# cinemere/evacuation

Measured on AMD Instinct MI355X. Metric: env-steps/s (agent-updates/s) at n=60x4096 envs, higher is better.
Workload: dtype f32

## Files before the change

evacuation_amd/csrc/evac_families.h:

```cpp
#pragma once

#include <type_traits>

#include "evac_common.h"

namespace evac {


template <int WPE_, int BLOCK1_ = 256>
struct Wave {
    static constexpr int WPE = WPE_;
    static constexpr bool kEnvUniform = true;
    static constexpr int kThreadsPerEnv = WPE * kWave;
    static constexpr int kBlock = (WPE == 1 || BLOCK1_ == 1024) ? (BLOCK1_ > kThreadsPerEnv ? BLOCK1_ : kThreadsPerEnv) : kThreadsPerEnv;
    static constexpr int kEnvsPerBlock = kBlock / kThreadsPerEnv;
    static constexpr bool kPace = kBlock == 1024 && kEnvsPerBlock > 1;
    static constexpr bool kEnvBarrier = WPE > 1 && kEnvsPerBlock > 1;
    static constexpr bool kHelpers = false, kExitLane = true, kPipelined = false;
    static constexpr const char* kName = WPE == 1 ? (kPace ? "1 wave/env, all pairs, CU-wide workgroups" : "1 wave/env, all pairs") : (WPE == 2 ? "2 waves/env, all pairs" : (WPE == 4 ? (kPace ? "4 waves/env, all pairs, CU-wide workgroups" : "4 waves/env, all pairs") : (WPE == 8 ? "8 waves/env, all pairs" : "16 waves/env, all pairs")));

    static constexpr int kTiles = WPE == 1 ? 1 : 2;
    static constexpr int kRows = WPE == 1 ? 1 : (WPE == 2 ? 2 : 4);
    static constexpr int kPairs = WPE * kWave / 2;

    struct Smem {
        f4 tile[kTiles][kEnvsPerBlock][WPE * kWave];
        float2 rowpos[kTiles][kEnvsPerBlock][WPE == 1 ? 1 : WPE * kWave];
        float2 part[kRows][kEnvsPerBlock][WPE == 1 ? 1 : WPE * kWave];
        f4 redf[kEnvsPerBlock][WPE];
        i4 redi[kEnvsPerBlock][WPE];
        int cols[kEnvsPerBlock][WPE];
        float exitg[kEnvsPerBlock][2];
        int poison[2][kEnvsPerBlock];
        int bar[kEnvsPerBlock];
        int persist_cmd[kEnvsPerBlock][6];
        alignas(16) float stage[kEnvsPerBlock][kStageSteps][12];
        alignas(16) int progress[kPace ? 16 : 4];
        int pace_sink[kPace ? 16 : 1][kPace ? kWave : 1];
        int deal_hist[kPace ? kWave + 2 : 1];
        int chain_ok[kEnvsPerBlock];
    };

    struct Ctx {
        using Family = Wave<WPE_, BLOCK1_>;
        Smem& sm;
        int env, slot, wave_in_env, lane, i;
        bool owner;
        int par = 0, next_cols = 0, next_base = 0, next_rows = 0, next_rbase = 0;
        bool have_next = false;
        __device__ __forceinline__ explicit Ctx(Smem& s) : sm(s) {
            const int t = threadIdx.x;
            slot = t / kThreadsPerEnv;
            const int tin = t - slot * kThreadsPerEnv;
            wave_in_env = tin / kWave;
            lane = tin & (kWave - 1);
            i = tin;
            env = blockIdx.x * kEnvsPerBlock + slot;
            if constexpr (WPE == 1) {
                env = __builtin_amdgcn_readfirstlane(env);
                slot = __builtin_amdgcn_readfirstlane(slot);
            }
            owner = i == 0;
        }
    };

    static __device__ __forceinline__ void sync() {
        static_assert(!kEnvBarrier, "several multi-wave envs per workgroup: use sync(ctx)");
        if constexpr (WPE == 1) {
            __builtin_amdgcn_fence(__ATOMIC_ACQ_REL, "wavefront");
            __builtin_amdgcn_wave_barrier();
        } else {
            __syncthreads();
        }
    }
    template <class C>
    static __device__ __forceinline__ void sync(C& c) {
        if constexpr (!kEnvBarrier) {
            sync();
        } else {
            __builtin_amdgcn_fence(__ATOMIC_RELEASE, "workgroup");
            if (c.lane == 0) {
                int* ctr = &c.sm.bar[c.slot];
                const int old = __hip_atomic_fetch_add(ctr, 1, __ATOMIC_RELAXED, __HIP_MEMORY_SCOPE_WORKGROUP);
                const int target = (old & ~(WPE - 1)) + WPE;
                int spins = 0;
                while (__hip_atomic_load(ctr, __ATOMIC_RELAXED, __HIP_MEMORY_SCOPE_WORKGROUP) < target && ++spins < (1 << 24)) __builtin_amdgcn_s_sleep(0);
            }
            __builtin_amdgcn_fence(__ATOMIC_ACQUIRE, "workgroup");
            __builtin_amdgcn_wave_barrier();
        }
    }

    static __device__ __forceinline__ void init(Ctx& c) {
        if constexpr (WPE > 1) {
            if (c.wave_in_env == 0 && c.lane < 2) c.sm.poison[c.lane][c.slot] = 0;
            if (c.wave_in_env == 0 && c.lane == 2) c.sm.bar[c.slot] = 0;
            __syncthreads();
        }
    }
    static __device__ __forceinline__ void invalidate(Ctx& c) { c.have_next = false; }
    static __device__ __forceinline__ bool aborted(Ctx&) { return false; }

    template <bool GUARD, class C>
    static __device__ __forceinline__ void reduce(const Params&, C& c, Sums& s, const unsigned long long (&pred)[8]) {
        wave_sum3(s.f0, s.f1, s.f2);
#pragma unroll
        for (int k = 0; k < 8; ++k) s.i[k] = mask_count(pred[k]);
        if constexpr (WPE > 1) {
            auto& sm = c.sm;
            if constexpr (GUARD) C::Family::sync(c);
            if (c.lane == 0) {
                sm.redf[c.slot][c.wave_in_env] = f4{s.f0, s.f1, s.f2, 0.0f};
                sm.redi[c.slot][c.wave_in_env] = i4{s.i[0] | (s.i[1] << 16), s.i[2] | (s.i[3] << 16), s.i[4] | (s.i[5] << 16), s.i[6] | (s.i[7] << 16)};
            }
            C::Family::sync(c);
            const int w = c.lane < WPE ? c.lane : WPE - 1;
            f4 rf = sm.redf[c.slot][w];
            i4 ri = sm.redi[c.slot][w];
#define EVAC_RED_STEP(CTRL)                                                                                      \
    rf.x = dpp_add<CTRL, 0xf>(rf.x); rf.y = dpp_add<CTRL, 0xf>(rf.y); rf.z = dpp_add<CTRL, 0xf>(rf.z);           \
    ri.x = dpp_addi<CTRL, 0xf>(ri.x); ri.y = dpp_addi<CTRL, 0xf>(ri.y); ri.z = dpp_addi<CTRL, 0xf>(ri.z);        \
    ri.w = dpp_addi<CTRL, 0xf>(ri.w);
            EVAC_RED_STEP(0x111)
            if constexpr (WPE > 2) { EVAC_RED_STEP(0x112) }
            if constexpr (WPE > 4) { EVAC_RED_STEP(0x114) }
            if constexpr (WPE > 8) { EVAC_RED_STEP(0x118) }
#undef EVAC_RED_STEP
            s.f0 = readlane_f(rf.x, WPE - 1);
            s.f1 = readlane_f(rf.y, WPE - 1);
            s.f2 = readlane_f(rf.z, WPE - 1);
            if constexpr (!GUARD && std::is_same<typename C::Family, Wave>::value) {
                const int wi = __builtin_amdgcn_readfirstlane(c.wave_in_env);
                const int before = wi == 0 ? 0 : __builtin_amdgcn_readlane(ri.y, max(wi - 1, 0));
                c.next_base = before >> 16;
                c.next_cols = __builtin_amdgcn_readlane(ri.y, WPE - 1) >> 16;
                const int rbefore = wi == 0 ? 0 : __builtin_amdgcn_readlane(ri.z, max(wi - 1, 0));
                c.next_rbase = rbefore >> 16;
                c.next_rows = __builtin_amdgcn_readlane(ri.z, WPE - 1) >> 16;
                c.have_next = true;
            }
            const int a = __builtin_amdgcn_readlane(ri.x, WPE - 1), b = __builtin_amdgcn_readlane(ri.y, WPE - 1);
            const int d = __builtin_amdgcn_readlane(ri.z, WPE - 1), g = __builtin_amdgcn_readlane(ri.w, WPE - 1);
            s.i[0] = a & 0xffff; s.i[1] = a >> 16;
            s.i[2] = b & 0xffff; s.i[3] = b >> 16;
            s.i[4] = d & 0xffff; s.i[5] = d >> 16;
            s.i[6] = g & 0xffff; s.i[7] = g >> 16;
        }
    }

    template <class C>
    static __device__ __forceinline__ void exit_publish(C& c, bool exit_lane, float gx, float gy) {
        if constexpr (WPE > 1) {
            if (exit_lane) {
                c.sm.exitg[c.slot][0] = gx;
                c.sm.exitg[c.slot][1] = gy;
            }
        }
    }
    template <class C>
    static __device__ __forceinline__ void exit_fetch(C& c, float gx, float gy, int src_i, float& ex, float& ey) {
        if constexpr (WPE == 1) {
            ex = readlane_f(gx, src_i);
            ey = readlane_f(gy, src_i);
        } else {
            ex = c.sm.exitg[c.slot][0];
            ey = c.sm.exitg[c.slot][1];
        }
    }

    static __device__ __forceinline__ void neighbour_sum(const Params& p, Ctx& c, const Ped& q, bool efv, bool fv,
                                                         float ux, float uy, float& sx, float& sy) {
        auto& sm = c.sm;
        int par = 0;
        if constexpr (WPE == 1) {
            sx = 0.0f;
            sy = 0.0f;
            if (ballot(fv) == 0ull) {
                if ((ballot(ux != ux || uy != uy) & ballot(efv)) != 0ull) sx = sy = __builtin_nanf("");
                return;
            }
            sync(c);
        } else {
            par = c.par;
            c.par = par ^ 1;
        }
        int n_cols, n_rows = 0, row_rank = 0;
        unsigned long long moving_mask;
        {
            const unsigned long long m = moving_mask = ballot(efv);
            int before = __builtin_amdgcn_mbcnt_hi((unsigned)(m >> 32), __builtin_amdgcn_mbcnt_lo((unsigned)m, 0u));
            n_cols = __popcll(m);
            if constexpr (WPE > 1) {
                const unsigned long long mr = ballot(fv);
                row_rank = __builtin_amdgcn_mbcnt_hi((unsigned)(mr >> 32), __builtin_amdgcn_mbcnt_lo((unsigned)mr, 0u));
                n_rows = __popcll(mr);
                if (c.have_next) {
                    n_cols = c.next_cols;
                    before += c.next_base;
                    n_rows = c.next_rows;
                    row_rank += c.next_rbase;
                } else {
                    if (c.lane == 0) sm.cols[c.slot][c.wave_in_env] = n_cols | (n_rows << 16);
                    sync(c);
                    int tot = 0, base = 0;
#pragma unroll
                    for (int w2 = 0; w2 < WPE; ++w2) {
                        const int k = sm.cols[c.slot][w2];
                        base += (w2 < c.wave_in_env) ? k : 0;
                        tot += k;
                    }
                    n_cols = tot & 0xffff;
                    before += base & 0xffff;
                    n_rows = tot >> 16;
                    row_rank += base >> 16;
                }
            }
            const int tid = c.wave_in_env * kWave + c.lane;
            const int idx = efv ? before : n_cols + (tid - before);
            if constexpr (WPE == 1) {
                float* tf = (float*)sm.tile[par][c.slot] + (idx >> 1) * 4 + (idx & 1);
                tf[0] = efv ? q.x * kTileScale : __builtin_inff();
                tf[2] = q.y * kTileScale;
                tf[kPairs * 4 + 0] = efv ? ux : 0.0f;
                tf[kPairs * 4 + 2] = efv ? uy : 0.0f;
            } else {
                sm.tile[par][c.slot][idx] = f4{efv ? q.x * kTileScale : __builtin_inff(), q.y * kTileScale, efv ? ux : 0.0f, efv ? uy : 0.0f};
            }
        }
        if constexpr (WPE > 1) {
            if (fv) sm.rowpos[par][c.slot][row_rank] = make_float2(q.x * kTileScale, q.y * kTileScale);
            if ((ballot(ux != ux || uy != uy) & moving_mask) != 0ull && c.lane == 0) sm.poison[par][c.slot] = 1;
        }
        sync(c);
        bool poisoned = false;
        if constexpr (WPE > 1) {
            poisoned = sm.poison[par][c.slot] != 0;
            if (c.wave_in_env == 0 && c.lane == 0) sm.poison[par ^ 1][c.slot] = 0;
        }
        sx = 0.0f;
        sy = 0.0f;
        const f4* __restrict__ tile = sm.tile[par][c.slot];
        const float r2b = kRPed2Big;
        if constexpr (WPE == 1) {
            const int n8 = __builtin_amdgcn_readfirstlane((n_cols + 3) & ~3);
            const float XI = q.x * kTileScale, YI = q.y * kTileScale;
            constexpr int B = 16;
            const f2 P = f2{XI, YI}, r2b2 = f2{r2b, r2b};
            f2 sx2 = f2{0.0f, 0.0f}, sy2 = f2{0.0f, 0.0f};
            const f4* __restrict__ txy = tile;
            const f4* __restrict__ tuv = tile + kPairs;
            int m = 0;
            const int mp = n8 >> 1;
            for (; m + B / 2 <= mp; m += B / 2) {
                f4 a[B / 2], u[B / 2];
#pragma unroll
                for (int k = 0; k < B / 2; ++k) { a[k] = txy[m + k]; u[k] = tuv[m + k]; }
#pragma unroll
                for (int k = 0; k < B / 2; ++k) pair2_accumulate(P, a[k], u[k], r2b2, sx2, sy2);
            }
            if (mp - m >= 4) {
                f4 a[4], u[4];
#pragma unroll
                for (int k = 0; k < 4; ++k) { a[k] = txy[m + k]; u[k] = tuv[m + k]; }
#pragma unroll
                for (int k = 0; k < 4; ++k) pair2_accumulate(P, a[k], u[k], r2b2, sx2, sy2);
                m += 4;
            }
            if (m < mp) {
                f4 a[2], u[2];
#pragma unroll
                for (int k = 0; k < 2; ++k) { a[k] = txy[m + k]; u[k] = tuv[m + k]; }
#pragma unroll
                for (int k = 0; k < 2; ++k) pair2_accumulate(P, a[k], u[k], r2b2, sx2, sy2);
            }
            sx = hsum2(sx2);
            sy = hsum2(sy2);
        } else {
            const unsigned wu = (unsigned)__builtin_amdgcn_readfirstlane(c.wave_in_env);
            const unsigned nc = (unsigned)__builtin_amdgcn_readfirstlane(n_cols), nr = (unsigned)__builtin_amdgcn_readfirstlane(n_rows);
            const unsigned share_u = wu % (unsigned)kRows, first_row = (wu - share_u) * (unsigned)kWave;
            const int share = (int)share_u, gbase = (int)first_row + c.lane;
            const int slices = nr > first_row ? (int)min((nr - first_row + (unsigned)kWave - 1u) / (unsigned)kWave, (unsigned)kRows) : 0;
            const unsigned groups = (nc + 3u) >> 2;
            const unsigned per = (groups + (unsigned)kRows - 1u) / (unsigned)kRows;
            const int jbeg = (int)(share_u * per * 4u);
            const int jend = (int)(min((share_u + 1u) * per, groups) * 4u);
            auto sweep = [&](auto r_tag) {
                constexpr int R = decltype(r_tag)::value;
                constexpr int R2 = R / 2;
                float X[R], Y[R], ax[R], ay[R];
                f2 X2[R2 ? R2 : 1], Y2[R2 ? R2 : 1], ax2[R2 ? R2 : 1], ay2[R2 ? R2 : 1];
#pragma unroll
                for (int r = 0; r < R; ++r) {
                    const float2 rp = sm.rowpos[par][c.slot][gbase + r * kWave];
                    X[r] = rp.x; Y[r] = rp.y;
                    ax[r] = 0.0f; ay[r] = 0.0f;
                }
#pragma unroll
                for (int r = 0; r < R2; ++r) {
                    X2[r] = f2{X[2 * r], X[2 * r + 1]}; Y2[r] = f2{Y[2 * r], Y[2 * r + 1]};
                    ax2[r] = f2{0.0f, 0.0f}; ay2[r] = f2{0.0f, 0.0f};
                }
                const f2 r2b2 = f2{r2b, r2b};
                auto column = [&](f4 t) {
#pragma unroll
                    for (int r = 0; r < R2; ++r) pair_accumulate_rows2(X2[r], Y2[r], t, r2b2, ax2[r], ay2[r]);
#pragma unroll
                    for (int r = 2 * R2; r < R; ++r) pair_accumulate(X[r], Y[r], t, r2b, ax[r], ay[r]);
                };
                constexpr int B = (R <= 2 && !(kEnvBarrier && R == 2)) ? 8 : 4;
                int j = jbeg;
                for (; j + B <= jend; j += B) {
                    f4 t[B];
#pragma unroll
                    for (int k = 0; k < B; ++k) t[k] = tile[j + k];
#pragma unroll
                    for (int k = 0; k < B; ++k) column(t[k]);
                }
                if constexpr (B == 8) {
                    if (j < jend) {
                        f4 t[4];
#pragma unroll
                        for (int k = 0; k < 4; ++k) t[k] = tile[j + k];
#pragma unroll
                        for (int k = 0; k < 4; ++k) column(t[k]);
                    }
                }
#pragma unroll
                for (int r = 0; r < R2; ++r) { ax[2 * r] = ax2[r].x; ax[2 * r + 1] = ax2[r].y; ay[2 * r] = ay2[r].x; ay[2 * r + 1] = ay2[r].y; }
#pragma unroll
                for (int r = 0; r < R; ++r) sm.part[share][c.slot][gbase + r * kWave] = make_float2(ax[r], ay[r]);
            };
            if (slices == 1) sweep(std::integral_constant<int, 1>{});
            else if (slices == 2) sweep(std::integral_constant<int, 2>{});
            else if constexpr (kRows == 4) {
                if (slices == 3) sweep(std::integral_constant<int, 3>{});
                else if (slices == 4) sweep(std::integral_constant<int, 4>{});
            }
            sync(c);
            if (fv) {
#pragma unroll
                for (int r = 0; r < kRows; ++r) {
                    const float2 pr = sm.part[r][c.slot][row_rank];
                    sx += pr.x;
                    sy += pr.y;
                }
            }
            if (poisoned) sx = sy = __builtin_nanf("");
        }
    }
};

template <int WPE_>
struct Cells {
    static constexpr int WPE = WPE_;
    static_assert(WPE >= 2, "Cells is a workgroup-per-env family");
    static constexpr bool kEnvUniform = true;
    static constexpr int kThreadsPerEnv = WPE * kWave;
    static constexpr int kBlock = kThreadsPerEnv;
    static constexpr int kEnvsPerBlock = 1;
    static constexpr bool kPace = false, kHelpers = false, kExitLane = true, kPipelined = false, kEnvBarrier = false;
    static constexpr int kPad = 8;
    static constexpr int kRowBatch = 8;
    static constexpr int kTransposedWork = 1024;
    static constexpr const char* kName = WPE == 2 ? "2 waves/env, cell list" : (WPE == 4 ? "4 waves/env, cell list" : (WPE == 8 ? "8 waves/env, cell list" : "16 waves/env, cell list"));

    struct Smem {
        f4 tile[1][kThreadsPerEnv + kPad];
        alignas(16) int cnt[kCells + 4];
        alignas(16) int start[kCells + 4];
        int who[kThreadsPerEnv];
        int rowlist[kThreadsPerEnv];
        i2 res[kThreadsPerEnv];
        char one_workgroup_per_cu[WPE == 16 ? 52 * 1024 : 16];
        f4 redf[1][WPE];
        i4 redi[1][WPE];
        float exitg[1][2];
        alignas(16) float stage[1][kStageSteps][12];
    };

    struct Ctx {
        using Family = Cells<WPE_>;
        Smem& sm;
        int env, slot, wave_in_env, lane, i;
        bool owner;
        __device__ __forceinline__ explicit Ctx(Smem& s) : sm(s) {
            const int t = threadIdx.x;
            slot = 0;
            wave_in_env = t / kWave;
            lane = t & (kWave - 1);
            i = t;
            env = blockIdx.x;
            owner = i == 0;
        }
    };

    static __device__ __forceinline__ void sync() { __syncthreads(); }
    template <class C>
    static __device__ __forceinline__ void sync(C&) { __syncthreads(); }

    static __device__ __forceinline__ void invalidate(Ctx&) {}
    static __device__ __forceinline__ bool aborted(Ctx&) { return false; }
    static __device__ __forceinline__ void init(Ctx& c) {
        for (int k = c.i; k < kCells + 4; k += kThreadsPerEnv) c.sm.cnt[k] = 0;
        __syncthreads();
    }

    template <bool GUARD, class C>
    static __device__ __forceinline__ void reduce(const Params& p, C& c, Sums& s, const unsigned long long (&pred)[8]) {
        Wave<WPE>::template reduce<GUARD>(p, c, s, pred);
    }
    template <class C>
    static __device__ __forceinline__ void exit_publish(C& c, bool exit_lane, float gx, float gy) {
        Wave<WPE>::exit_publish(c, exit_lane, gx, gy);
    }
    template <class C>
    static __device__ __forceinline__ void exit_fetch(C& c, float gx, float gy, int src_i, float& ex, float& ey) {
        Wave<WPE>::exit_fetch(c, gx, gy, src_i, ex, ey);
    }

    static __device__ __forceinline__ int cell_of(const Params& p, float x, float y) {
        int cx = (int)((x + p.cell_ox) * p.cell_inv_hx), cy = (int)((y + p.cell_oy) * p.cell_inv_hy);
        cx = min(max(cx, 0), kCellsX - 1);
        cy = min(max(cy, 0), kCellsY - 1);
        return cx * kCellsY + cy;
    }

    static __device__ __forceinline__ void neighbour_sum(const Params& p, Ctx& c, const Ped& q, bool efv, bool fv,
                                                         float ux, float uy, float& sx, float& sy) {
        auto& sm = c.sm;
        const int cell = cell_of(p, q.x, q.y);
        int ticket = 0;
        if (efv) {
            ticket = atomicAdd(&sm.cnt[cell], 1);
            if (ux != ux || uy != uy) atomicAdd(&sm.cnt[kCells], 1);
        }
        __syncthreads();
        if (c.wave_in_env == 0) {
            const i4 v = *(const i4*)&sm.cnt[4 * c.lane];
            const int p1 = v.x, p2 = p1 + v.y, p3 = p2 + v.z, tot = p3 + v.w;
            const int incl = wave_inclusive_scan(tot);
            const int ex = incl - tot;
            *(i4*)&sm.start[4 * c.lane] = i4{ex, ex + p1, ex + p2, ex + p3};
            *(i4*)&sm.cnt[4 * c.lane] = i4{0, 0, 0, 0};
            if (c.lane == kWave - 1) {
                sm.start[kCells] = incl;
                sm.start[kCells + 1] = sm.cnt[kCells];
                sm.cnt[kCells] = 0;
                sm.cnt[kCells + 1] = 0;
            }
        }
        __syncthreads();
        const int n_cols = sm.start[kCells];
        const int n_nan = sm.start[kCells + 1];
        if (efv) {
            const int s = sm.start[cell] + ticket;
            const float hs = p.head_scale;
            const int hx = (int)__builtin_rintf(ux * hs), hy = (int)__builtin_rintf(uy * hs);
            sm.tile[0][s] = f4{q.x * kTileScale, q.y * kTileScale, __builtin_bit_cast(float, hx), __builtin_bit_cast(float, hy)};
            sm.who[s] = c.i | (fv ? 0x8000 : 0) | (cell << 16);
            if (fv) sm.rowlist[atomicAdd(&sm.cnt[kCells + 1], 1)] = s;
        }
        if (c.i < kPad) sm.tile[0][n_cols + c.i] = f4{__builtin_inff(), 0.0f, 0.0f, 0.0f};
        __syncthreads();
        const int n_need = __builtin_amdgcn_readfirstlane(sm.cnt[kCells + 1]);
        const int n_cols_u = __builtin_amdgcn_readfirstlane(n_cols);
        const bool transposed = n_need * ((n_cols_u + kWave - 1) / kWave) <= kTransposedWork;
          if (transposed) {
            const f4* __restrict__ tile = sm.tile[0];
            const int wv = __builtin_amdgcn_readfirstlane(c.wave_in_env);
            for (int k = wv; k < n_need; k += WPE) {
                const int s = sm.rowlist[k];
                const f4 me = tile[s];
                const int ped = sm.who[s] & 0x7fff;
                int ax = 0, ay = 0;
                for (int j0 = 0; j0 < n_cols_u; j0 += kWave)
                    pair_accumulate_int(me.x, me.y, tile[min(j0 + c.lane, n_cols_u)], kRPed2Big, ax, ay);
                wave_sum2_int_lane63(ax, ay);
                if (c.lane == kWave - 1) sm.res[ped] = i2{ax, ay};
            }
          } else {
            const int s = c.i;
            const int wc = s < n_cols ? sm.who[s] : 0;
            if (wc & 0x8000) {
                const f4 me = sm.tile[0][s];
                const int rc = wc >> 16;
                int lo[3], hi[3];
#pragma unroll
                for (int r = 0; r < 3; ++r) {
                    const int c0 = rc + (r - 1) * kCellsY - 1;
                    lo[r] = sm.start[min(max(c0, 0), kCells)];
                    hi[r] = sm.start[min(max(c0 + 3, 0), kCells)];
                }
                int ax = 0, ay = 0;
                int j = lo[0];
                const f4* __restrict__ tile = sm.tile[0];
#pragma unroll
                for (int r = 0; r < 3; ++r) {
                    j = max(j, lo[r]);
                    while (j < hi[r]) {
                        f4 t[kRowBatch];
#pragma unroll
                        for (int k = 0; k < kRowBatch; ++k) t[k] = tile[j + k];
#pragma unroll
                        for (int k = 0; k < kRowBatch; ++k) pair_accumulate_int(me.x, me.y, t[k], kRPed2Big, ax, ay);
                        j += kRowBatch;
                    }
                }
                sm.res[wc & 0x7fff] = i2{ax, ay};
            }
          }
        __syncthreads();
        const i2 r = sm.res[c.i];
        sx = fv ? (float)r.x : 0.0f;
        sy = fv ? (float)r.y : 0.0f;
        if (n_nan != 0) sx = sy = __builtin_nanf("");
    }
};

template <int G_, int BLOCK_ = 256>
struct Sub {
    static constexpr int G = G_;
    static_assert(G == 16 || G == 32, "sub-wave groups are 16 or 32 lanes");
    static constexpr bool kEnvUniform = false, kHelpers = false, kExitLane = true, kPipelined = false, kEnvBarrier = false;
    static constexpr int kThreadsPerEnv = G;
    static constexpr int kEnvsPerWave = kWave / G;
    static constexpr int kBlock = BLOCK_;
    static constexpr int kEnvsPerBlock = (kBlock / kWave) * kEnvsPerWave;
    static constexpr unsigned long long kGroupBits = G == 32 ? 0xffffffffull : 0xffffull;
    static constexpr const char* kName = G == 16 ? "4 envs/wave, all pairs" : "2 envs/wave, all pairs";

    struct Smem {
        f4 tile[kEnvsPerBlock][G];
    };

    struct Ctx {
        Smem& sm;
        int env, slot, lane, sub, i, li;
        unsigned long long gmask;
        bool owner;
        __device__ __forceinline__ explicit Ctx(Smem& s) : sm(s) {
            const int t = threadIdx.x;
            lane = t & (kWave - 1);
            sub = lane / G;
            li = i = lane - sub * G;
            slot = (t / kWave) * kEnvsPerWave + sub;
            env = blockIdx.x * kEnvsPerBlock + slot;
            gmask = kGroupBits << (sub * G);
            owner = li == G - 1;
        }
    };

    static __device__ __forceinline__ void sync() {
        __builtin_amdgcn_fence(__ATOMIC_ACQ_REL, "wavefront");
        __builtin_amdgcn_wave_barrier();
    }
    static __device__ __forceinline__ int count(unsigned long long m, unsigned long long gmask) { return __popcll(m & gmask); }
    static __device__ __forceinline__ int rank(unsigned long long m, unsigned long long gmask) {
        const unsigned long long g = m & gmask;
        return __builtin_amdgcn_mbcnt_hi((unsigned)(g >> 32), __builtin_amdgcn_mbcnt_lo((unsigned)g, 0u));
    }
    static __device__ __forceinline__ float fetch(float v, int sub_base, int src_i) { return __shfl(v, sub_base + src_i, kWave); }

    static __device__ __forceinline__ void invalidate(Ctx&) {}
    static __device__ __forceinline__ bool aborted(Ctx&) { return false; }
    template <bool GUARD, class C>
    static __device__ __forceinline__ void reduce(const Params&, C& c, Sums& s, const unsigned long long (&pred)[8]) {
        float &a = s.f0, &b = s.f1, &cc = s.f2;
        {
            float& c = cc;
            EVAC_DPP3(0x111, 0xf)
            EVAC_DPP3(0x112, 0xf)
            EVAC_DPP3(0x114, 0xf)
            EVAC_DPP3(0x118, 0xf)
            if constexpr (G == 32) { EVAC_DPP3(0x142, 0xa) }
        }
#pragma unroll
        for (int k = 0; k < 8; ++k) s.i[k] = count(pred[k], c.gmask);
    }
    template <class C>
    static __device__ __forceinline__ void exit_publish(C&, bool, float, float) {}
    template <class C>
    static __device__ __forceinline__ void exit_fetch(C& c, float gx, float gy, int src_i, float& ex, float& ey) {
        ex = fetch(gx, c.sub * G, src_i);
        ey = fetch(gy, c.sub * G, src_i);
    }

    static __device__ __forceinline__ void neighbour_sum(const Params& p, Ctx& c, const Ped& q, bool efv, bool fv,
                                                         float ux, float uy, float& sx, float& sy) {
        auto& sm = c.sm;
        sync();
        const unsigned long long m_efv = ballot(efv);
        const int n_cols = count(m_efv, c.gmask);
        {
            const int before = rank(m_efv, c.gmask);
            const int idx = efv ? before : n_cols + (c.li - before);
            float* tf = (float*)sm.tile[c.slot] + (idx >> 1) * 8 + (idx & 1);
            tf[0] = efv ? q.x * kTileScale : __builtin_inff();
            tf[2] = q.y * kTileScale;
            tf[4] = efv ? ux : 0.0f;
            tf[6] = efv ? uy : 0.0f;
        }
        sync();
        sx = 0.0f;
        sy = 0.0f;
        int nmax = 0;
#pragma unroll
        for (int g = 0; g < kEnvsPerWave; ++g) {
            const int k = __popcll((m_efv >> (g * G)) & kGroupBits);
            nmax = k > nmax ? k : nmax;
        }
        const bool any_row = ballot(fv) != 0ull;
        const int n4 = any_row ? ((nmax + 3) & ~3) : 0;
        if (!any_row) {
            const unsigned long long m_nan = ballot(ux != ux || uy != uy) & m_efv;
            if ((m_nan & c.gmask) != 0ull) sx = sy = __builtin_nanf("");
        }
        const f4* __restrict__ tile = sm.tile[c.slot];
        const float XI = q.x * kTileScale, YI = q.y * kTileScale;
        int j = 0;
        const f2 P = f2{XI, YI}, r2b2 = f2{kRPed2Big, kRPed2Big};
        f2 sx2 = f2{0.0f, 0.0f}, sy2 = f2{0.0f, 0.0f};
        for (; j + 8 <= n4; j += 8) {
            f4 t[8];
#pragma unroll
            for (int k = 0; k < 8; ++k) t[k] = tile[j + k];
#pragma unroll
            for (int k = 0; k < 8; k += 2) pair2_accumulate(P, t[k], t[k + 1], r2b2, sx2, sy2);
        }
        for (; j < n4; j += 4) {
            f4 t[4];
#pragma unroll
            for (int k = 0; k < 4; ++k) t[k] = tile[j + k];
#pragma unroll
            for (int k = 0; k < 4; k += 2) pair2_accumulate(P, t[k], t[k + 1], r2b2, sx2, sy2);
        }
        if (any_row) {
            sx = sx2.x + sx2.y;
            sy = sy2.x + sy2.y;
        }
    }
};

}
```

Baseline: 704.3 million.

## Hand-schedule WPE=1 pair sweep with inline asm LDS reads and lgkmcnt waits

Replaces the compiler-generated WPE=1 all-pairs loop with inline assembly. It issues ds_read_b128 loads in batches and waits on lgkmcnt, so the packed FMA math on one group overlaps the LDS reads of the next. The pair math is rewritten as hand-scheduled v_pk_add/v_pk_fma sequences that use clamp to form the weight, and the loop is fully unrolled up to four batches of eight pairs with static remainder dispatch. This risks hardcoding the limit of at most 32 pair groups, and it leaves the compiler unaware of these register and LDS dependencies.

```diff
diff --git a/evacuation_amd/csrc/evac_families.h b/evacuation_amd/csrc/evac_families.h
--- a/evacuation_amd/csrc/evac_families.h
+++ b/evacuation_amd/csrc/evac_families.h
@@ -6,6 +6,60 @@
 
 namespace evac {
 
+
+template <int N>
+__device__ __forceinline__ void wait_lgkm() { __builtin_amdgcn_s_waitcnt(0xC07F | (N << 8)); }
+__device__ __forceinline__ void pair2_accumulate_group(f2 P, f4 xy0, f4 uv0, f4 xy1, f4 uv1, f2 r2b2, f2& sx2, f2& sy2) {
+    f2 t0, t1, t2, t3;
+    asm volatile(
+        "v_pk_add_f32 %1, %6, %8 op_sel:[1,0] op_sel_hi:[1,1] neg_lo:[0,1] neg_hi:[0,1]\n\t"
+        "v_pk_add_f32 %0, %6, %7 op_sel_hi:[0,1] neg_lo:[0,1] neg_hi:[0,1]\n\t"
+        "v_pk_add_f32 %3, %6, %10 op_sel:[1,0] op_sel_hi:[1,1] neg_lo:[0,1] neg_hi:[0,1]\n\t"
+        "v_pk_fma_f32 %1, %1, %1, %15 neg_lo:[1,0,0] neg_hi:[1,0,0]\n\t"
+        "v_pk_add_f32 %2, %6, %9 op_sel_hi:[0,1] neg_lo:[0,1] neg_hi:[0,1]\n\t"
+        "v_pk_fma_f32 %3, %3, %3, %15 neg_lo:[1,0,0] neg_hi:[1,0,0]\n\t"
+        "v_pk_fma_f32 %0, %0, %0, %1 neg_lo:[1,0,0] neg_hi:[1,0,0] clamp\n\t"
+        "v_pk_fma_f32 %2, %2, %2, %3 neg_lo:[1,0,0] neg_hi:[1,0,0] clamp\n\t"
+        "v_pk_fma_f32 %4, %0, %11, %4\n\t"
+        "v_pk_fma_f32 %5, %0, %12, %5\n\t"
+        "v_pk_fma_f32 %4, %2, %13, %4\n\t"
+        "v_pk_fma_f32 %5, %2, %14, %5"
+        : "=&v"(t0), "=&v"(t1), "=&v"(t2), "=&v"(t3), "+v"(sx2), "+v"(sy2)
+        : "v"(P), "v"(__builtin_shufflevector(xy0, xy0, 0, 1)), "v"(__builtin_shufflevector(xy0, xy0, 2, 3)),
+          "v"(__builtin_shufflevector(xy1, xy1, 0, 1)), "v"(__builtin_shufflevector(xy1, xy1, 2, 3)),
+          "v"(__builtin_shufflevector(uv0, uv0, 0, 1)), "v"(__builtin_shufflevector(uv0, uv0, 2, 3)),
+          "v"(__builtin_shufflevector(uv1, uv1, 0, 1)), "v"(__builtin_shufflevector(uv1, uv1, 2, 3)), "s"(r2b2));
+}
+template <int PAIR, int kUv>
+__device__ __forceinline__ void pair_group_read(unsigned lds, f4& xy0, f4& xy1, f4& uv0, f4& uv1) {
+    asm volatile("ds_read_b128 %0, %4 offset:%5\n\tds_read_b128 %1, %4 offset:%6\n\tds_read_b128 %2, %4 offset:%7\n\tds_read_b128 %3, %4 offset:%8"
+                 : "=&v"(xy0), "=&v"(xy1), "=&v"(uv0), "=&v"(uv1)
+                 : "v"(lds), "n"(16 * PAIR), "n"(16 * (PAIR + 1)), "n"(kUv + 16 * PAIR), "n"(kUv + 16 * (PAIR + 1))
+                 : "memory");
+}
+template <int G, int PAIR0, int kUv>
+__device__ __forceinline__ void pair_batch(f2 P, unsigned lds, f2 r2b2, f2& sx2, f2& sy2) {
+    static_assert(G >= 1 && G <= 4, "lgkmcnt counts to 15");
+    f4 a[8], u[8];
+    pair_group_read<PAIR0, kUv>(lds, a[0], a[1], u[0], u[1]);
+    if constexpr (G >= 2) pair_group_read<PAIR0 + 2, kUv>(lds, a[2], a[3], u[2], u[3]);
+    if constexpr (G >= 3) pair_group_read<PAIR0 + 4, kUv>(lds, a[4], a[5], u[4], u[5]);
+    wait_lgkm<4 * ((G < 3 ? G : 3) - 1)>();
+    pair2_accumulate_group(P, a[0], u[0], a[1], u[1], r2b2, sx2, sy2);
+    if constexpr (G == 4) pair_group_read<PAIR0 + 6, kUv>(lds, a[6], a[7], u[6], u[7]);
+    if constexpr (G >= 2) {
+        wait_lgkm<4 * (G - 2)>();
+        pair2_accumulate_group(P, a[2], u[2], a[3], u[3], r2b2, sx2, sy2);
+    }
+    if constexpr (G >= 3) {
+        wait_lgkm<4 * (G - 3)>();
+        pair2_accumulate_group(P, a[4], u[4], a[5], u[5], r2b2, sx2, sy2);
+    }
+    if constexpr (G == 4) {
+        wait_lgkm<0>();
+        pair2_accumulate_group(P, a[6], u[6], a[7], u[7], r2b2, sx2, sy2);
+    }
+}
 
 template <int WPE_, int BLOCK1_ = 256>
 struct Wave {
@@ -249,30 +303,26 @@
             f2 sx2 = f2{0.0f, 0.0f}, sy2 = f2{0.0f, 0.0f};
             const f4* __restrict__ txy = tile;
             const f4* __restrict__ tuv = tile + kPairs;
-            int m = 0;
-            const int mp = n8 >> 1;
-            for (; m + B / 2 <= mp; m += B / 2) {
-                f4 a[B / 2], u[B / 2];
-#pragma unroll
-                for (int k = 0; k < B / 2; ++k) { a[k] = txy[m + k]; u[k] = tuv[m + k]; }
-#pragma unroll
-                for (int k = 0; k < B / 2; ++k) pair2_accumulate(P, a[k], u[k], r2b2, sx2, sy2);
-            }
-            if (mp - m >= 4) {
-                f4 a[4], u[4];
-#pragma unroll
-                for (int k = 0; k < 4; ++k) { a[k] = txy[m + k]; u[k] = tuv[m + k]; }
-#pragma unroll
-                for (int k = 0; k < 4; ++k) pair2_accumulate(P, a[k], u[k], r2b2, sx2, sy2);
-                m += 4;
-            }
-            if (m < mp) {
-                f4 a[2], u[2];
-#pragma unroll
-                for (int k = 0; k < 2; ++k) { a[k] = txy[m + k]; u[k] = tuv[m + k]; }
-#pragma unroll
-                for (int k = 0; k < 2; ++k) pair2_accumulate(P, a[k], u[k], r2b2, sx2, sy2);
-            }
+            const int mp = n8 >> 1, nb = mp >> 3;
+            constexpr int kUv = kPairs * 16;
+            const unsigned lds = (unsigned)(unsigned long long)(__attribute__((address_space(3))) const f4*)txy;
+            if (nb >= 1) {
+                pair_batch<4, 0, kUv>(P, lds, r2b2, sx2, sy2);
+                if (nb >= 2) {
+                    pair_batch<4, 8, kUv>(P, lds, r2b2, sx2, sy2);
+                    if (nb >= 3) {
+                        pair_batch<4, 16, kUv>(P, lds, r2b2, sx2, sy2);
+                        if (nb >= 4) pair_batch<4, 24, kUv>(P, lds, r2b2, sx2, sy2);
+                    }
+                }
+            }
+            const int rest = mp & 7;
+            const unsigned rl = lds + (unsigned)(mp - rest) * 16u;
+            int rest4 = rest, rest2 = rest;
+            asm("" : "+s"(rest4), "+s"(rest2));
+            if (rest == 6) pair_batch<3, 0, kUv>(P, rl, r2b2, sx2, sy2);
+            if (rest4 == 4) pair_batch<2, 0, kUv>(P, rl, r2b2, sx2, sy2);
+            if (rest2 == 2) pair_batch<1, 0, kUv>(P, rl, r2b2, sx2, sy2);
             sx = hsum2(sx2);
             sy = hsum2(sy2);
         } else {
```

Result: slower. 524.0 million (-25.6%).
